# KorAP/Datok

Measured on AMD Instinct MI355X. Metric: input MB/s tokenized, tokenizer_de.matok, higher is better.
Workload: dtype u32 table cells, u8 symbol codes; 1 GPU; tokenizer_de.matok, 4096 equal-length 4096 B synthetic German docs per batch (BASELINE.json configs[1]); table_layout=matrix: state-major fused u32 cells, docs_per_gpu=4096, doc_bytes=4096, parallelism=documents sharded over 1 GPU(s), no data-path collective, batches_in_flight=3, inputs=one per batch in flight (generator seeds 2, 3, 4 on rank 0)

## Files before the change

### datok_amd/csrc/dtk_symbolize.hip

```cpp
#include "dtk_device.h"

__device__ __forceinline__ uint32_t go_width(uint32_t b0, uint32_t b1, uint32_t b2, uint32_t b3, uint32_t avail) {
  const uint32_t c1 = (b1 & 0xC0u) == 0x80u, c2 = (b2 & 0xC0u) == 0x80u, c3 = (b3 & 0xC0u) == 0x80u;
  const uint32_t two = (uint32_t)(b0 - 0xC2u < 0x1Eu) & (uint32_t)(avail >= 2u) & c1;
  const uint32_t lo3 = b0 == 0xE0u ? 0xA0u : 0x80u, hi3 = b0 == 0xEDu ? 0x9Fu : 0xBFu;
  const uint32_t three = (uint32_t)((b0 & 0xF0u) == 0xE0u) & (uint32_t)(avail >= 3u) & (uint32_t)(b1 >= lo3) &
                         (uint32_t)(b1 <= hi3) & c2;
  const uint32_t lo4 = b0 == 0xF0u ? 0x90u : 0x80u, hi4 = b0 == 0xF4u ? 0x8Fu : 0xBFu;
  const uint32_t four = (uint32_t)(b0 - 0xF0u <= 4u) & (uint32_t)(avail >= 4u) & (uint32_t)(b1 >= lo4) &
                        (uint32_t)(b1 <= hi4) & c2 & c3;
  return 1u + two + 2u * three + 3u * four;
}


#define SYM_BLOCK_BYTES DTK_SYM_BLOCK_BYTES
#define SYM_SIG_LDS 64u
#define SYM_HALF 1024u
#define SYM_THREADS (WAVE * (SYM_BLOCK_BYTES / SYM_HALF))
#define SYM_DOFF (SYM_BLOCK_BYTES / 16u)
#define SYM_FAR 0x10000u

__device__ __forceinline__ void sym_clear_acc(uint4 *__restrict__ acc, uint32_t acc16) {
  if (!acc) return;
  const uint4 z = make_uint4(0u, 0u, 0u, 0u);
  constexpr uint32_t kept16 = offsetof(DtkTotalsDev, invalid_epoch) / 16u;
  constexpr uint32_t flags8 = offsetof(DtkTotalsDev, any_irregular) / 8u;
  for (uint32_t i = blockIdx.x * SYM_THREADS + threadIdx.x; i < acc16; i += gridDim.x * SYM_THREADS) {
    if (i == kept16) reinterpret_cast<unsigned long long *>(acc)[flags8] = 0ull;
    else acc[i] = z;
  }
}

__device__ __forceinline__ void sym_clear_events(uint32_t *__restrict__ ev_bits, uint32_t bit_words, uint64_t block_start,
                                                 uint32_t n_here, uint32_t d_lo, uint32_t d_hi) {
  if (!ev_bits) return;
  const uint64_t ga = block_start + d_lo, gb = block_start + n_here + d_hi + 1u;
  const uint32_t wa = blockIdx.x == 0 ? 0u : (uint32_t)(ga >> 5);
  uint32_t wb = (uint32_t)((gb + 31u) >> 5);
  if (wb > bit_words || blockIdx.x == gridDim.x - 1) wb = bit_words;
  for (uint32_t w = wa + threadIdx.x; w < wb; w += SYM_THREADS)
#pragma unroll
    for (uint32_t k = 0; k < EVB_KINDS; k++) ev_bits[(size_t)k * bit_words + w] = 0u;
}

__device__ __forceinline__ void sym_saw_invalid(bool bad, unsigned long long *__restrict__ n_invalid, unsigned long long epoch) {
  if (__ballot(bad) != 0ull && lane_id() == 0 &&
      __hip_atomic_load(n_invalid, __ATOMIC_RELAXED, __HIP_MEMORY_SCOPE_AGENT) != epoch)
    atomicMax(n_invalid, epoch);
}


__device__ __forceinline__ uint32_t sym_gather7(uint32_t x) {
  uint32_t t = x & 0x80808080u;
  t |= t << 7;
  t |= t << 14;
  return t >> 28;
}
__device__ __forceinline__ uint32_t sym_bytes_of7(uint32_t m) { return (m << 1) - (m >> 7); }
__device__ __forceinline__ uint32_t sym_spread7(uint32_t nib) {
  uint32_t t = nib | (nib << 7);
  t |= t << 14;
  return (t & 0x01010101u) << 7;
}
__device__ __forceinline__ uint32_t sym_window(uint32_t w0, uint32_t w1, uint32_t w2, uint32_t w3, uint32_t nx,
                                                        uint32_t p) {
  const bool k1 = (p & 4u) != 0u, k2 = (p & 8u) != 0u;
  const uint32_t lo = k2 ? (k1 ? w3 : w2) : (k1 ? w1 : w0), hi = k2 ? (k1 ? nx : w3) : (k1 ? w2 : w1);
  return __builtin_amdgcn_alignbyte(hi, lo, p & 3u);
}
__device__ __forceinline__ void sym_patch(uint32_t &w0, uint32_t &w1, uint32_t &w2, uint32_t &w3, uint32_t p,
                                                   uint32_t code) {
  const uint32_t sh = 8u * (p & 3u), keep = ~(0xFFu << sh), c = code << sh, k = p >> 2;
  w0 = k == 0u ? (w0 & keep) | c : w0;
  w1 = k == 1u ? (w1 & keep) | c : w1;
  w2 = k == 2u ? (w2 & keep) | c : w2;
  w3 = k == 3u ? (w3 & keep) | c : w3;
}
__device__ __forceinline__ uint32_t sym_rune(uint32_t x, uint32_t w) {
  const uint32_t b0 = x & 0xFFu, b1 = (x >> 8) & 0x3Fu, b2 = (x >> 16) & 0x3Fu, b3 = (x >> 24) & 0x3Fu;
  const uint32_t r2 = ((b0 & 0x1Fu) << 6) | b1;
  const uint32_t r3 = ((b0 & 0x0Fu) << 12) | (b1 << 6) | b2;
  const uint32_t r4 = ((b0 & 0x07u) << 18) | (b1 << 12) | (b2 << 6) | b3;
  return w == 2u ? r2 : (w == 3u ? r3 : r4);
}

template <bool ALIGNED4>
__global__ __launch_bounds__(SYM_THREADS) void k_symbolize8(const uint8_t *__restrict__ text,
                                                     const uint64_t *__restrict__ doc_off,
                                                     uint32_t n_docs, uint64_t total, DtkSigmaDev sig,
                                                     uint8_t *__restrict__ sym8,
                                                     const uint32_t *__restrict__ blk_doc,
                                                     unsigned long long *__restrict__ n_invalid,
                                                     uint32_t *__restrict__ rs_bits,
                                                     uint32_t *__restrict__ ev_bits, uint32_t bit_words,
                                                     uint4 *__restrict__ acc, uint32_t acc16,
                                                     unsigned long long epoch) {
  sym_clear_acc(acc, acc16);
  __shared__ uint32_t s_lat[64];
  __shared__ uint32_t s_runes[SYM_SIG_LDS];
  __shared__ uint8_t s_codes[SYM_SIG_LDS];
  __shared__ uint64_t s_doff[SYM_DOFF];
  const uint32_t tid = threadIdx.x, lane = tid & (WAVE - 1u);
  const uint64_t block_start = (uint64_t)blockIdx.x * SYM_BLOCK_BYTES;
  const uint32_t n_here = (uint32_t)min((uint64_t)SYM_BLOCK_BYTES, total - block_start);
  const uint32_t i0 = tid * 16u;
  const uint64_t g0 = block_start + i0;

  auto load4 = [&](uint64_t g) -> uint32_t {
    uint32_t x = 0;
    if (ALIGNED4) {
      if (g < total) {
        x = *reinterpret_cast<const uint32_t *>(text + g);
        if (total - g < 4u) x &= (1u << (8u * (uint32_t)(total - g))) - 1u;
      }
    } else {
      for (int k = 0; k < 4; k++)
        if (g + k < total) x |= (uint32_t)text[g + k] << (8 * k);
    }
    return x;
  };
  uint32_t w0, w1, w2, w3, halo = 0;
  if (ALIGNED4 && total - block_start >= SYM_BLOCK_BYTES + 4u) {
    const uint32_t *t4 = reinterpret_cast<const uint32_t *>(text + g0);
    w0 = t4[0]; w1 = t4[1]; w2 = t4[2]; w3 = t4[3];
    if (lane == 0 && g0 >= 4u) halo = t4[-1];
    if (lane == WAVE - 1u) halo = t4[4];
  } else {
    w0 = load4(g0); w1 = load4(g0 + 4u); w2 = load4(g0 + 8u); w3 = load4(g0 + 12u);
    if (lane == 0 && g0 >= 4u) halo = load4(g0 - 4u);
    if (lane == WAVE - 1u) halo = load4(g0 + 16u);
  }

  const bool sig_lds = sig.n_runes < SYM_SIG_LDS;
  if (tid < 64u) s_lat[tid] = reinterpret_cast<const uint32_t *>(sig.code_lt256)[tid];
  if (sig_lds && tid < SYM_SIG_LDS) {
    s_runes[tid] = tid < sig.n_runes ? sig.runes[tid] : 0xFFFFFFFFu;
    if (tid < sig.n_runes) s_codes[tid] = sig.code_runes[tid];
  }
  const uint32_t d_lo = blk_doc[blockIdx.x];
  const uint32_t d_hi = min(blk_doc[blockIdx.x + 1], n_docs - 1);
  const uint32_t n_off = d_hi - d_lo + 2u;
  if (n_off <= SYM_DOFF && tid < n_off) s_doff[tid] = doc_off[d_lo + tid];
  const uint64_t lo_start = doc_off[d_lo], lo_end = doc_off[d_lo + 1];
  const uint32_t lo_end_rel = (uint32_t)min(lo_end - block_start, (uint64_t)SYM_FAR);
  sym_clear_events(ev_bits, bit_words, block_start, n_here, d_lo, d_hi);
  __syncthreads();

  if ((tid & ~(WAVE - 1u)) * 16u >= n_here) return;
  auto doc_end_rel = [&](uint32_t pos) -> uint32_t {
    const uint64_t g = block_start + pos;
    uint64_t dend;
    if (n_off <= SYM_DOFF) {
      uint32_t lo = 0, hi = n_off - 1u;
      while (hi - lo > 1u) {
        const uint32_t mid = lo + ((hi - lo) >> 1);
        if (s_doff[mid] <= g) lo = mid; else hi = mid;
      }
      dend = s_doff[lo + 1u];
    } else {
      dend = doc_off[doc_of(doc_off, d_lo, d_hi + 1, g) + 1u];
    }
    return (uint32_t)min(dend - block_start, (uint64_t)SYM_FAR);
  };

  const uint32_t nval = i0 < n_here ? min(n_here - i0, 16u) : 0u;
  uint32_t covered = 0;
  if (__ballot(((w0 | w1 | w2 | w3) & 0x80808080u) != 0u) != 0ull) {
    const uint32_t nx = (uint32_t)__builtin_amdgcn_update_dpp((int)halo, (int)w0, 0x130, 0xF, 0xF, false);
    const uint32_t hi16 = sym_gather7(w0) | (sym_gather7(w1) << 4) | (sym_gather7(w2) << 8) | (sym_gather7(w3) << 12);
    uint32_t lead = sym_gather7(w0 & (w0 << 1)) | (sym_gather7(w1 & (w1 << 1)) << 4) |
                    (sym_gather7(w2 & (w2 << 1)) << 8) | (sym_gather7(w3 & (w3 << 1)) << 12);
    const uint32_t cont16 = hi16 & ~lead;
    const uint32_t c0 = w0 & ~(w0 << 1) & 0x80808080u, c1 = w1 & ~(w1 << 1) & 0x80808080u,
                   c2 = w2 & ~(w2 << 1) & 0x80808080u, c3 = w3 & ~(w3 << 1) & 0x80808080u;
    const uint32_t invalid_code = sig.code_fffd1;
    bool bad = false;
    uint32_t dend = lo_end_rel;
    auto width_at = [&](uint32_t x, uint32_t pos) -> uint32_t {
      if (pos >= dend) dend = doc_end_rel(pos);
      return go_width(x & 0xFFu, (x >> 8) & 0xFFu, (x >> 16) & 0xFFu, x >> 24, min(dend - pos, 4u));
    };
    uint32_t spill0 = 0;
    if (lane == 0 && (cont16 & 1u) && g0 >= 4u) {
      const uint32_t k = halo >= 0xC0000000u ? 1u : ((halo & 0x00C00000u) == 0x00C00000u ? 2u : ((halo & 0x0000C000u) == 0x0000C000u ? 3u : 0u));
      if (k) {
        const uint32_t x = __builtin_amdgcn_alignbyte(w0, halo, 4u - k);
        const uint64_t g = g0 - k;
        uint64_t de = lo_end;
        if (g < lo_start) de = doc_off[doc_of(doc_off, 0, d_lo, g) + 1u];
        else if (g >= lo_end) de = block_start + doc_end_rel(i0 - k);
        const uint32_t w = go_width(x & 0xFFu, (x >> 8) & 0xFFu, (x >> 16) & 0xFFu, x >> 24, (uint32_t)min(de - g, (uint64_t)4u));
        spill0 = w > k ? (1u << (w - k)) - 1u : 0u;
      }
    }
    for (; __builtin_amdgcn_ballot_w64(lead != 0u) != 0ull; lead &= lead - 1u) {
      if (lead == 0u) continue;
      const uint32_t p = (uint32_t)__builtin_ctz(lead);
      const uint32_t x = sym_window(w0, w1, w2, w3, nx, p);
      const uint32_t w = width_at(x, i0 + p);
      uint32_t code = invalid_code;
      if (w >= 2u) {
        const uint32_t rune = sym_rune(x, w);
        if (rune < 256u) {
          code = (s_lat[rune >> 2] >> (8u * (rune & 3u))) & 0xFFu;
        } else {
          code = w == 2u ? sig.code_ident[2] : (w == 3u ? sig.code_ident[3] : sig.code_ident[4]);
          if (sig_lds) {
            uint32_t n = 0;
#pragma unroll
            for (uint32_t step = SYM_SIG_LDS / 2u; step; step >>= 1) n += s_runes[n + step - 1u] <= rune ? step : 0u;
            if (n && s_runes[n - 1u] == rune) code = s_codes[n - 1u];
          } else {
            uint32_t base = 0;
            for (uint32_t len = sig.n_runes; len > 1u;) {
              const uint32_t half = len >> 1;
              base = sig.runes[base + half] <= rune ? base + half : base;
              len -= half;
            }
            if (sig.runes[base] == rune) code = sig.code_runes[base];
          }
        }
      }
      sym_patch(w0, w1, w2, w3, p, code);
      covered |= ((1u << w) - 2u) << p;
      bad |= w == 1u;
    }
    uint32_t spill = (uint32_t)__builtin_amdgcn_update_dpp(0, (int)(covered >> 16), 0x138, 0xF, 0xF, false);
    if (lane == 0) spill = spill0;
    covered = (covered | spill) & 0xFFFFu;
    static_assert(DTK_SYM_CONT == 0xFFu, "a continuation byte becomes DTK_SYM_CONT by setting all its bits");
    w0 |= sym_bytes_of7(c0); w1 |= sym_bytes_of7(c1); w2 |= sym_bytes_of7(c2); w3 |= sym_bytes_of7(c3);
    const uint32_t stray = cont16 & ~covered;
    if (__ballot(stray != 0u) != 0ull) {
      const uint32_t flip = (DTK_SYM_CONT ^ invalid_code) * 0x01010101u;
      w0 ^= sym_bytes_of7(sym_spread7(stray & 15u)) & flip;
      w1 ^= sym_bytes_of7(sym_spread7((stray >> 4) & 15u)) & flip;
      w2 ^= sym_bytes_of7(sym_spread7((stray >> 8) & 15u)) & flip;
      w3 ^= sym_bytes_of7(sym_spread7(stray >> 12)) & flip;
      bad |= stray != 0u;
    }
    sym_saw_invalid(bad, n_invalid, epoch);
  }

  if (nval == 16u && ((reinterpret_cast<uintptr_t>(sym8) + block_start) & 15u) == 0) {
    *reinterpret_cast<uint4 *>(sym8 + g0) = make_uint4(w0, w1, w2, w3);
  } else {
#pragma unroll
    for (uint32_t j = 0; j < 16u; j++) {
      const uint32_t wj = j < 4u ? w0 : (j < 8u ? w1 : (j < 12u ? w2 : w3));
      if (j < nval) sym8[g0 + j] = (uint8_t)(wj >> (8u * (j & 3u)));
    }
  }
  const uint32_t starts = ((1u << nval) - 1u) & ~covered;
  const uint32_t upper = (uint32_t)__builtin_amdgcn_update_dpp(0, (int)starts, 0x101, 0xF, 0xF, true);
  if (!(lane & 1u) && nval) rs_bits[(block_start >> 5) + (tid >> 1)] = starts | (upper << 16);
}

#define SYM_TILE 512u

template <bool ALIGNED4>
__global__ __launch_bounds__(SYM_THREADS) void k_symbolize16(const uint8_t *__restrict__ text,
                                                    const uint64_t *__restrict__ doc_off,
                                                    uint32_t n_docs, uint64_t total, DtkSigmaDev sig,
                                                    uint16_t *__restrict__ sym,
                                                    const uint32_t *__restrict__ blk_doc,
                                                    unsigned long long *__restrict__ n_invalid,
                                                    uint32_t *__restrict__ rs_bits,
                                                    uint32_t *__restrict__ ev_bits, uint32_t bit_words,
                                                    uint4 *__restrict__ acc, uint32_t acc16,
                                                    unsigned long long epoch) {
  sym_clear_acc(acc, acc16);
  __shared__ uint32_t s_rs[SYM_BLOCK_BYTES / 32];
  __shared__ uint16_t lut[128];
  __shared__ uint16_t lat[256];
  __shared__ uint32_t s_runes[SYM_SIG_LDS];
  __shared__ uint16_t s_syms[SYM_SIG_LDS];
  __shared__ uint32_t s_txt[SYM_BLOCK_BYTES / 4 + 4];
  __shared__ uint16_t s_qs[SYM_BLOCK_BYTES / SYM_HALF][SYM_HALF];
  __shared__ uint64_t s_doff[SYM_DOFF];
  const uint32_t tid = threadIdx.x, lane = tid & (WAVE - 1u), half = tid >> 6;
  uint16_t *s_q = s_qs[half];
  const bool sig_lds = sig.n_runes <= SYM_SIG_LDS;
  for (uint32_t i = tid; i < SYM_BLOCK_BYTES / 32; i += SYM_THREADS) s_rs[i] = 0;
  for (uint32_t i = tid; i < 256u; i += SYM_THREADS) {
    const uint32_t e = (sig.ascii[i] & DTK_SYM_MASK) | (i == DTK_EOT ? (1u << DTK_SYM_CLS_SHIFT) : 0u);
    lat[i] = (uint16_t)e;
    if (i < 128u) lut[i] = (uint16_t)(e | (1u << DTK_SYM_W_SHIFT));
    if (sig_lds && i < sig.n_runes) { s_runes[i] = sig.runes[i]; s_syms[i] = sig.syms[i]; }
  }
  const uint64_t block_start = (uint64_t)blockIdx.x * SYM_BLOCK_BYTES;
  const uint32_t n_here = (uint32_t)min((uint64_t)SYM_BLOCK_BYTES, total - block_start);
  const uint32_t d_lo = blk_doc[blockIdx.x];
  const uint32_t d_hi = min(blk_doc[blockIdx.x + 1], n_docs - 1);
  const uint32_t n_off = d_hi - d_lo + 2u;
  if (n_off <= SYM_DOFF && tid < n_off) s_doff[tid] = doc_off[d_lo + tid];
  {
    auto load4 = [&](uint64_t g) -> uint32_t {
      if (ALIGNED4) return g < total ? *reinterpret_cast<const uint32_t *>(text + g) : 0u;
      uint32_t x = 0;
      for (int k = 0; k < 4; k++)
        if (g + k < total) x |= (uint32_t)text[g + k] << (8 * k);
      return x;
    };
    uint32_t v[SYM_BLOCK_BYTES / 4 / SYM_THREADS];
#pragma unroll
    for (uint32_t r = 0; r < SYM_BLOCK_BYTES / 4 / SYM_THREADS; r++) v[r] = load4(block_start + (r * SYM_THREADS + tid) * 4u);
    uint32_t halo = 0;
    if (tid == 0 && block_start >= 4) halo = load4(block_start - 4);
    if (tid == 1) halo = load4(block_start + SYM_BLOCK_BYTES);
#pragma unroll
    for (uint32_t r = 0; r < SYM_BLOCK_BYTES / 4 / SYM_THREADS; r++) s_txt[1 + r * SYM_THREADS + tid] = v[r];
    if (tid == 0) s_txt[0] = halo;
    if (tid == 1) s_txt[1 + SYM_BLOCK_BYTES / 4] = halo;
  }
  __syncthreads();
  const uint8_t *__restrict__ sb = reinterpret_cast<const uint8_t *>(s_txt) + 4;

  const uint64_t lo_start = doc_off[d_lo], lo_end = doc_off[d_lo + 1];
  sym_clear_events(ev_bits, bit_words, block_start, n_here, d_lo, d_hi);
  const bool sym16 = ((reinterpret_cast<uintptr_t>(sym) + 2ull * block_start) & 15u) == 0;

  if (half * SYM_HALF < n_here) {
    uint32_t qn = 0;
    auto light = [&](auto full_tag, uint32_t it) {
      constexpr bool FULL = decltype(full_tag)::value;
      const uint32_t i0 = half * SYM_HALF + it * SYM_TILE + lane * 8u;
      const uint32_t w0 = s_txt[1 + (i0 >> 2)], w1 = s_txt[2 + (i0 >> 2)];
      uint32_t left = 8u;
      if (!FULL) left = i0 < n_here ? (n_here - i0 >= 8u ? 8u : n_here - i0) : 0u;
      const uint32_t e0 = lut[w0 & 0x7Fu], e1 = lut[(w0 >> 8) & 0x7Fu];
      const uint32_t e2 = lut[(w0 >> 16) & 0x7Fu], e3 = lut[(w0 >> 24) & 0x7Fu];
      const uint32_t e4 = lut[w1 & 0x7Fu], e5 = lut[(w1 >> 8) & 0x7Fu];
      const uint32_t e6 = lut[(w1 >> 16) & 0x7Fu], e7 = lut[(w1 >> 24) & 0x7Fu];
      if (FULL || (left == 8u && sym16)) {
        *reinterpret_cast<uint4 *>(sym + block_start + i0) =
            make_uint4(e0 | (e1 << 16), e2 | (e3 << 16), e4 | (e5 << 16), e6 | (e7 << 16));
      } else {
        const uint32_t o[8] = {e0, e1, e2, e3, e4, e5, e6, e7};
        for (uint32_t j = 0; j < left; j++) sym[block_start + i0 + j] = (uint16_t)o[j];
      }
      auto nib = [](uint32_t x) { return ((x >> 7) & 1u) | ((x >> 14) & 2u) | ((x >> 21) & 4u) | ((x >> 28) & 8u); };
      const uint32_t valid = FULL ? 0xFFu : ((1u << left) - 1u);
      const uint32_t rare = (nib(w0 & 0x80808080u) | (nib(w1 & 0x80808080u) << 4)) & valid;
      const uint32_t asc = ~rare & valid;
      if (asc) atomicOr(&s_rs[i0 >> 5], asc << (i0 & 31u));
      const uint32_t cnt = (uint32_t)__popc(rare);
      const unsigned long long b0 = __ballot(cnt & 1u), b1 = __ballot(cnt & 2u), b2 = __ballot(cnt & 4u),
                               b3 = __ballot(cnt & 8u);
      if ((b0 | b1 | b2 | b3) == 0ull) return;
      const unsigned long long lt = lanemask_lt();
      uint32_t slot = qn + popc(b0 & lt) + 2u * popc(b1 & lt) + 4u * popc(b2 & lt) + 8u * popc(b3 & lt);
      qn += popc(b0) + 2u * popc(b1) + 4u * popc(b2) + 8u * popc(b3);
      for (uint32_t m = rare; __builtin_amdgcn_ballot_w64(m != 0u) != 0ull; m &= m - 1u)
        if (m) s_q[slot++] = (uint16_t)(i0 + (uint32_t)__builtin_ctz(m));
    };
    const bool full_block = n_here == SYM_BLOCK_BYTES && sym16;
#pragma unroll 1
    for (uint32_t it = 0; it < SYM_HALF / SYM_TILE; it++) {
      if (half * SYM_HALF + it * SYM_TILE >= n_here) break;
      if (full_block) light(std::true_type{}, it); else light(std::false_type{}, it);
    }
    __builtin_amdgcn_fence(__ATOMIC_ACQ_REL, "wavefront");
    __builtin_amdgcn_wave_barrier();
    const uint32_t nq = qn;
    if (nq) __builtin_amdgcn_s_waitcnt(0);

    for (uint32_t q0 = 0; q0 < nq; q0 += WAVE) {
      bool bad = false;
      if (q0 + lane < nq) {
        const uint32_t pos = s_q[q0 + lane];
        const uint64_t g = block_start + pos;
        uint64_t dstart = lo_start, dend = lo_end;
        if (g >= lo_end) {
          if (n_off <= SYM_DOFF) {
            uint32_t lo = 0, hi = n_off - 1u;
            while (hi - lo > 1u) {
              const uint32_t mid = lo + ((hi - lo) >> 1);
              if (s_doff[mid] <= g) lo = mid; else hi = mid;
            }
            dstart = s_doff[lo]; dend = s_doff[lo + 1u];
          } else {
            const uint32_t d = doc_of(doc_off, d_lo, d_hi + 1, g);
            dstart = doc_off[d]; dend = doc_off[d + 1];
          }
        }
        const uint64_t l64 = dend - g, b64 = g - dstart;
        const uint32_t avail = l64 > 8 ? 8u : (uint32_t)l64, back = b64 > 3 ? 3u : (uint32_t)b64;
        uint32_t bb[7];
#pragma unroll
        for (int k = 0; k < 7; k++) {
          const int o = k - 3;
          const bool in = o < 0 ? (uint32_t)(-o) <= back : (uint32_t)o < avail;
          bb[k] = in ? (uint32_t)sb[(int)pos + o] : 0u;
        }
        const uint32_t b0 = bb[3], b1 = bb[4], b2 = bb[5], b3 = bb[6];
        const uint32_t n1 = (uint32_t)((bb[2] & 0xC0u) != 0x80u), n2 = (uint32_t)((bb[1] & 0xC0u) != 0x80u),
                       n3 = (uint32_t)((bb[0] & 0xC0u) != 0x80u);
        const uint32_t in1 = (uint32_t)(back >= 1u), in2 = (uint32_t)(back >= 2u), in3 = (uint32_t)(back >= 3u);
        const uint32_t cont = (uint32_t)((b0 & 0xC0u) == 0x80u);
        const uint32_t k1 = cont & in1 & n1, k2 = cont & in2 & (n1 ^ 1u) & n2, k3 = cont & in3 & (n1 ^ 1u) & (n2 ^ 1u) & n3;
        const uint32_t k = k1 + 2u * k2 + 3u * k3;
        const uint32_t c0 = k3 ? bb[0] : (k2 ? bb[1] : (k1 ? bb[2] : b0)), c1 = k3 ? bb[1] : (k2 ? bb[2] : (k1 ? b0 : b1));
        const uint32_t c2 = k3 ? bb[2] : (k2 ? b0 : (k1 ? b1 : b2)), c3 = k3 ? b0 : (k2 ? b1 : (k1 ? b2 : b3));
        const uint32_t wseq = go_width(c0, c1, c2, c3, avail + k);
        const uint32_t start = k ? (uint32_t)(wseq <= k) : 1u;
        const uint32_t wd = cont ? 1u : wseq;
        const uint32_t r2 = ((b0 & 0x1Fu) << 6) | (b1 & 0x3Fu);
        const uint32_t r3 = ((b0 & 0x0Fu) << 12) | ((b1 & 0x3Fu) << 6) | (b2 & 0x3Fu);
        const uint32_t r4 = ((b0 & 0x07u) << 18) | ((b1 & 0x3Fu) << 12) | ((b2 & 0x3Fu) << 6) | (b3 & 0x3Fu);
        const uint32_t rune = wd == 1 ? 0xFFFDu : (wd == 2 ? r2 : (wd == 3 ? r3 : r4));
        uint32_t a_cls;
        if (rune < 256u) {
          a_cls = lat[rune];
        } else {
          int l = 0, h = (int)sig.n_runes - 1;
          a_cls = (sig.identity & DTK_SYM_MASK) | (3u << DTK_SYM_CLS_SHIFT);
          while (l <= h) {
            const int m = (l + h) >> 1;
            const uint32_t r = sig_lds ? s_runes[m] : sig.runes[m];
            if (r == rune) {
              a_cls = ((sig_lds ? (uint32_t)s_syms[m] : (uint32_t)sig.syms[m]) & DTK_SYM_MASK) | (2u << DTK_SYM_CLS_SHIFT);
              break;
            }
            if (r < rune) l = m + 1; else h = m - 1;
          }
        }
        sym[g] = (uint16_t)(a_cls | (start ? wd << DTK_SYM_W_SHIFT : 0u));
        if (start) atomicOr(&s_rs[pos >> 5], 1u << (pos & 31u));
        bad = start && wd == 1u;
      }
      sym_saw_invalid(bad, n_invalid, epoch);
    }
  }
  __syncthreads();
  for (uint32_t i = tid; i < SYM_BLOCK_BYTES / 32; i += SYM_THREADS)
    if (i * 32u < n_here) rs_bits[(block_start >> 5) + i] = s_rs[i];
}


extern "C" int dtk_launch_symbolize(const uint8_t *text, const uint64_t *doc_off, uint32_t n_docs,
                                    uint64_t total, const DtkSigmaDev *sig, void *sym, int padded,
                                    const uint32_t *blk_doc, unsigned long long *n_invalid, uint32_t *rs_bits,
                                    uint32_t *ev_bits, uint32_t bit_words, void *acc, uint64_t acc_bytes,
                                    uint64_t epoch, void *stream) {
  if (total == 0 || n_docs == 0) return 0;
  const uint32_t blocks = (uint32_t)((total + SYM_BLOCK_BYTES - 1) / SYM_BLOCK_BYTES);
  const bool al4 = (((uintptr_t)text) & 3u) == 0 && (padded || (total & 3u) == 0);
  auto go = [&](auto k, auto *out) {
    hipLaunchKernelGGL(k, dim3(blocks), dim3(SYM_THREADS), 0, (hipStream_t)stream, text, doc_off, n_docs,
                       total, *sig, out, blk_doc, n_invalid, rs_bits, ev_bits, bit_words, (uint4 *)acc, (uint32_t)(acc_bytes / 16),
                       (unsigned long long)epoch);
  };
  if (sig->n_codes) { if (al4) go(k_symbolize8<true>, (uint8_t *)sym); else go(k_symbolize8<false>, (uint8_t *)sym); }
  else { if (al4) go(k_symbolize16<true>, (uint16_t *)sym); else go(k_symbolize16<false>, (uint16_t *)sym); }
  return (int)hipGetLastError();
}
```

Baseline: 191,400 MB/s.

## Widen symbolize8 to 32 bytes per lane with a wave-uniform two-byte fast path

The 8-bit symbolize kernel now has each lane process 32 input bytes instead of 16, which halves the thread count per block and lets each lane write its rs_bits word directly instead of combining two lanes through DPP. The lead-byte loop adds a path for iterations where every pending lane has a valid two-byte UTF-8 sequence, skipping the full width and rune decode. The patch and continuation-byte masking helpers are simplified into XOR and multiply-free forms. The cost is higher register pressure and longer per-lane serial loops over lead bytes, which may reduce occupancy and latency hiding.

```diff
diff --git a/datok_amd/csrc/dtk_symbolize.hip b/datok_amd/csrc/dtk_symbolize.hip
--- a/datok_amd/csrc/dtk_symbolize.hip
+++ b/datok_amd/csrc/dtk_symbolize.hip
@@ -17,20 +17,25 @@
 #define SYM_SIG_LDS 64u
 #define SYM_HALF 1024u
 #define SYM_THREADS (WAVE * (SYM_BLOCK_BYTES / SYM_HALF))
+#define SYM8_LANE 32u
+#define SYM8_WAVE (WAVE * SYM8_LANE)
+#define SYM8_THREADS (WAVE * (SYM_BLOCK_BYTES / SYM8_WAVE))
 #define SYM_DOFF (SYM_BLOCK_BYTES / 16u)
 #define SYM_FAR 0x10000u
 
+template <uint32_t THREADS = SYM_THREADS>
 __device__ __forceinline__ void sym_clear_acc(uint4 *__restrict__ acc, uint32_t acc16) {
   if (!acc) return;
   const uint4 z = make_uint4(0u, 0u, 0u, 0u);
   constexpr uint32_t kept16 = offsetof(DtkTotalsDev, invalid_epoch) / 16u;
   constexpr uint32_t flags8 = offsetof(DtkTotalsDev, any_irregular) / 8u;
-  for (uint32_t i = blockIdx.x * SYM_THREADS + threadIdx.x; i < acc16; i += gridDim.x * SYM_THREADS) {
+  for (uint32_t i = blockIdx.x * THREADS + threadIdx.x; i < acc16; i += gridDim.x * THREADS) {
     if (i == kept16) reinterpret_cast<unsigned long long *>(acc)[flags8] = 0ull;
     else acc[i] = z;
   }
 }
 
+template <uint32_t THREADS = SYM_THREADS>
 __device__ __forceinline__ void sym_clear_events(uint32_t *__restrict__ ev_bits, uint32_t bit_words, uint64_t block_start,
                                                  uint32_t n_here, uint32_t d_lo, uint32_t d_hi) {
   if (!ev_bits) return;
@@ -38,7 +43,7 @@
   const uint32_t wa = blockIdx.x == 0 ? 0u : (uint32_t)(ga >> 5);
   uint32_t wb = (uint32_t)((gb + 31u) >> 5);
   if (wb > bit_words || blockIdx.x == gridDim.x - 1) wb = bit_words;
-  for (uint32_t w = wa + threadIdx.x; w < wb; w += SYM_THREADS)
+  for (uint32_t w = wa + threadIdx.x; w < wb; w += THREADS)
 #pragma unroll
     for (uint32_t k = 0; k < EVB_KINDS; k++) ev_bits[(size_t)k * bit_words + w] = 0u;
 }
@@ -56,25 +61,24 @@
   t |= t << 14;
   return t >> 28;
 }
-__device__ __forceinline__ uint32_t sym_bytes_of7(uint32_t m) { return (m << 1) - (m >> 7); }
-__device__ __forceinline__ uint32_t sym_spread7(uint32_t nib) {
+__device__ __forceinline__ uint32_t sym_bytes_of4(uint32_t nib) {
   uint32_t t = nib | (nib << 7);
   t |= t << 14;
-  return (t & 0x01010101u) << 7;
-}
-__device__ __forceinline__ uint32_t sym_window(uint32_t w0, uint32_t w1, uint32_t w2, uint32_t w3, uint32_t nx,
-                                                        uint32_t p) {
-  const bool k1 = (p & 4u) != 0u, k2 = (p & 8u) != 0u;
-  const uint32_t lo = k2 ? (k1 ? w3 : w2) : (k1 ? w1 : w0), hi = k2 ? (k1 ? nx : w3) : (k1 ? w2 : w1);
+  t &= 0x01010101u;
+  return (t << 8) - t;
+}
+__device__ __forceinline__ uint32_t sym_window(const uint32_t (&w)[8], uint32_t nx, uint32_t p) {
+  const bool k4 = (p & 16u) != 0u, k2 = (p & 8u) != 0u, k1 = (p & 4u) != 0u;
+  const uint32_t a0 = k4 ? w[4] : w[0], a1 = k4 ? w[5] : w[1], a2 = k4 ? w[6] : w[2], a3 = k4 ? w[7] : w[3],
+                 a4 = k4 ? nx : w[4];
+  const uint32_t b0 = k2 ? a2 : a0, b1 = k2 ? a3 : a1, b2 = k2 ? a4 : a2;
+  const uint32_t lo = k1 ? b1 : b0, hi = k1 ? b2 : b1;
   return __builtin_amdgcn_alignbyte(hi, lo, p & 3u);
 }
-__device__ __forceinline__ void sym_patch(uint32_t &w0, uint32_t &w1, uint32_t &w2, uint32_t &w3, uint32_t p,
-                                                   uint32_t code) {
-  const uint32_t sh = 8u * (p & 3u), keep = ~(0xFFu << sh), c = code << sh, k = p >> 2;
-  w0 = k == 0u ? (w0 & keep) | c : w0;
-  w1 = k == 1u ? (w1 & keep) | c : w1;
-  w2 = k == 2u ? (w2 & keep) | c : w2;
-  w3 = k == 3u ? (w3 & keep) | c : w3;
+__device__ __forceinline__ void sym_patch(uint32_t (&w)[8], uint32_t p, uint32_t was, uint32_t code) {
+  const uint32_t flip = (was ^ code) << (8u * (p & 3u)), k = p >> 2;
+#pragma unroll
+  for (uint32_t j = 0; j < 8u; j++) w[j] ^= k == j ? flip : 0u;
 }
 __device__ __forceinline__ uint32_t sym_rune(uint32_t x, uint32_t w) {
   const uint32_t b0 = x & 0xFFu, b1 = (x >> 8) & 0x3Fu, b2 = (x >> 16) & 0x3Fu, b3 = (x >> 24) & 0x3Fu;
@@ -85,7 +89,7 @@
 }
 
 template <bool ALIGNED4>
-__global__ __launch_bounds__(SYM_THREADS) void k_symbolize8(const uint8_t *__restrict__ text,
+__global__ __launch_bounds__(SYM8_THREADS) void k_symbolize8(const uint8_t *__restrict__ text,
                                                      const uint64_t *__restrict__ doc_off,
                                                      uint32_t n_docs, uint64_t total, DtkSigmaDev sig,
                                                      uint8_t *__restrict__ sym8,
@@ -95,7 +99,7 @@
                                                      uint32_t *__restrict__ ev_bits, uint32_t bit_words,
                                                      uint4 *__restrict__ acc, uint32_t acc16,
                                                      unsigned long long epoch) {
-  sym_clear_acc(acc, acc16);
+  sym_clear_acc<SYM8_THREADS>(acc, acc16);
   __shared__ uint32_t s_lat[64];
   __shared__ uint32_t s_runes[SYM_SIG_LDS];
   __shared__ uint8_t s_codes[SYM_SIG_LDS];
@@ -103,7 +107,7 @@
   const uint32_t tid = threadIdx.x, lane = tid & (WAVE - 1u);
   const uint64_t block_start = (uint64_t)blockIdx.x * SYM_BLOCK_BYTES;
   const uint32_t n_here = (uint32_t)min((uint64_t)SYM_BLOCK_BYTES, total - block_start);
-  const uint32_t i0 = tid * 16u;
+  const uint32_t i0 = tid * SYM8_LANE;
   const uint64_t g0 = block_start + i0;
 
   auto load4 = [&](uint64_t g) -> uint32_t {
@@ -119,16 +123,18 @@
     }
     return x;
   };
-  uint32_t w0, w1, w2, w3, halo = 0;
+  uint32_t w[8], halo = 0;
   if (ALIGNED4 && total - block_start >= SYM_BLOCK_BYTES + 4u) {
     const uint32_t *t4 = reinterpret_cast<const uint32_t *>(text + g0);
-    w0 = t4[0]; w1 = t4[1]; w2 = t4[2]; w3 = t4[3];
+#pragma unroll
+    for (uint32_t j = 0; j < 8u; j++) w[j] = t4[j];
     if (lane == 0 && g0 >= 4u) halo = t4[-1];
-    if (lane == WAVE - 1u) halo = t4[4];
+    if (lane == WAVE - 1u) halo = t4[8];
   } else {
-    w0 = load4(g0); w1 = load4(g0 + 4u); w2 = load4(g0 + 8u); w3 = load4(g0 + 12u);
+#pragma unroll
+    for (uint32_t j = 0; j < 8u; j++) w[j] = load4(g0 + 4u * j);
     if (lane == 0 && g0 >= 4u) halo = load4(g0 - 4u);
-    if (lane == WAVE - 1u) halo = load4(g0 + 16u);
+    if (lane == WAVE - 1u) halo = load4(g0 + SYM8_LANE);
   }
 
   const bool sig_lds = sig.n_runes < SYM_SIG_LDS;
@@ -140,13 +146,17 @@
   const uint32_t d_lo = blk_doc[blockIdx.x];
   const uint32_t d_hi = min(blk_doc[blockIdx.x + 1], n_docs - 1);
   const uint32_t n_off = d_hi - d_lo + 2u;
-  if (n_off <= SYM_DOFF && tid < n_off) s_doff[tid] = doc_off[d_lo + tid];
+  static_assert(SYM_DOFF == 2u * SYM8_THREADS, "two offsets per thread fill s_doff");
+  if (n_off <= SYM_DOFF) {
+    if (tid < n_off) s_doff[tid] = doc_off[d_lo + tid];
+    if (tid + SYM8_THREADS < n_off) s_doff[tid + SYM8_THREADS] = doc_off[d_lo + tid + SYM8_THREADS];
+  }
   const uint64_t lo_start = doc_off[d_lo], lo_end = doc_off[d_lo + 1];
   const uint32_t lo_end_rel = (uint32_t)min(lo_end - block_start, (uint64_t)SYM_FAR);
-  sym_clear_events(ev_bits, bit_words, block_start, n_here, d_lo, d_hi);
+  sym_clear_events<SYM8_THREADS>(ev_bits, bit_words, block_start, n_here, d_lo, d_hi);
   __syncthreads();
 
-  if ((tid & ~(WAVE - 1u)) * 16u >= n_here) return;
+  if ((tid & ~(WAVE - 1u)) * SYM8_LANE >= n_here) return;
   auto doc_end_rel = [&](uint32_t pos) -> uint32_t {
     const uint64_t g = block_start + pos;
     uint64_t dend;
@@ -163,97 +173,118 @@
     return (uint32_t)min(dend - block_start, (uint64_t)SYM_FAR);
   };
 
-  const uint32_t nval = i0 < n_here ? min(n_here - i0, 16u) : 0u;
-  uint32_t covered = 0;
-  if (__ballot(((w0 | w1 | w2 | w3) & 0x80808080u) != 0u) != 0ull) {
-    const uint32_t nx = (uint32_t)__builtin_amdgcn_update_dpp((int)halo, (int)w0, 0x130, 0xF, 0xF, false);
-    const uint32_t hi16 = sym_gather7(w0) | (sym_gather7(w1) << 4) | (sym_gather7(w2) << 8) | (sym_gather7(w3) << 12);
-    uint32_t lead = sym_gather7(w0 & (w0 << 1)) | (sym_gather7(w1 & (w1 << 1)) << 4) |
-                    (sym_gather7(w2 & (w2 << 1)) << 8) | (sym_gather7(w3 & (w3 << 1)) << 12);
-    const uint32_t cont16 = hi16 & ~lead;
-    const uint32_t c0 = w0 & ~(w0 << 1) & 0x80808080u, c1 = w1 & ~(w1 << 1) & 0x80808080u,
-                   c2 = w2 & ~(w2 << 1) & 0x80808080u, c3 = w3 & ~(w3 << 1) & 0x80808080u;
+  const uint32_t nval = i0 < n_here ? min(n_here - i0, SYM8_LANE) : 0u;
+  unsigned long long covered = 0;
+  uint32_t any = 0;
+#pragma unroll
+  for (uint32_t j = 0; j < 8u; j++) any |= w[j];
+  if (__ballot((any & 0x80808080u) != 0u) != 0ull) {
+    const uint32_t nx = (uint32_t)__builtin_amdgcn_update_dpp((int)halo, (int)w[0], 0x130, 0xF, 0xF, false);
+    uint32_t hi32 = 0, lead = 0;
+#pragma unroll
+    for (uint32_t j = 0; j < 8u; j++) {
+      hi32 |= sym_gather7(w[j]) << (4u * j);
+      lead |= sym_gather7(w[j] & (w[j] << 1)) << (4u * j);
+    }
+    const uint32_t cont32 = hi32 & ~lead;
     const uint32_t invalid_code = sig.code_fffd1;
     bool bad = false;
     uint32_t dend = lo_end_rel;
-    auto width_at = [&](uint32_t x, uint32_t pos) -> uint32_t {
-      if (pos >= dend) dend = doc_end_rel(pos);
-      return go_width(x & 0xFFu, (x >> 8) & 0xFFu, (x >> 16) & 0xFFu, x >> 24, min(dend - pos, 4u));
+    auto code_ge256 = [&](uint32_t rune, uint32_t ident) -> uint32_t {
+      uint32_t code = ident;
+      if (sig_lds) {
+        uint32_t n = 0;
+#pragma unroll
+        for (uint32_t step = SYM_SIG_LDS / 2u; step; step >>= 1) n += s_runes[n + step - 1u] <= rune ? step : 0u;
+        if (n && s_runes[n - 1u] == rune) code = s_codes[n - 1u];
+      } else {
+        uint32_t base = 0;
+        for (uint32_t len = sig.n_runes; len > 1u;) {
+          const uint32_t half = len >> 1;
+          base = sig.runes[base + half] <= rune ? base + half : base;
+          len -= half;
+        }
+        if (sig.runes[base] == rune) code = sig.code_runes[base];
+      }
+      return code;
     };
     uint32_t spill0 = 0;
-    if (lane == 0 && (cont16 & 1u) && g0 >= 4u) {
+    if (lane == 0 && (cont32 & 1u) && g0 >= 4u) {
       const uint32_t k = halo >= 0xC0000000u ? 1u : ((halo & 0x00C00000u) == 0x00C00000u ? 2u : ((halo & 0x0000C000u) == 0x0000C000u ? 3u : 0u));
       if (k) {
-        const uint32_t x = __builtin_amdgcn_alignbyte(w0, halo, 4u - k);
+        const uint32_t x = __builtin_amdgcn_alignbyte(w[0], halo, 4u - k);
         const uint64_t g = g0 - k;
         uint64_t de = lo_end;
         if (g < lo_start) de = doc_off[doc_of(doc_off, 0, d_lo, g) + 1u];
         else if (g >= lo_end) de = block_start + doc_end_rel(i0 - k);
-        const uint32_t w = go_width(x & 0xFFu, (x >> 8) & 0xFFu, (x >> 16) & 0xFFu, x >> 24, (uint32_t)min(de - g, (uint64_t)4u));
-        spill0 = w > k ? (1u << (w - k)) - 1u : 0u;
-      }
-    }
-    for (; __builtin_amdgcn_ballot_w64(lead != 0u) != 0ull; lead &= lead - 1u) {
+        const uint32_t wd = go_width(x & 0xFFu, (x >> 8) & 0xFFu, (x >> 16) & 0xFFu, x >> 24, (uint32_t)min(de - g, (uint64_t)4u));
+        spill0 = wd > k ? (1u << (wd - k)) - 1u : 0u;
+      }
+    }
+    for (;; lead &= lead - 1u) {
+      uint32_t p = 0, x = 0, avail = 0;
+      bool two = false;
+      if (lead != 0u) {
+        p = (uint32_t)__builtin_ctz(lead);
+        x = sym_window(w, nx, p);
+        if (i0 + p >= dend) dend = doc_end_rel(i0 + p);
+        avail = min(dend - (i0 + p), 4u);
+        two = ((x & 0xFFu) - 0xC2u < 0x1Eu) & ((x & 0xC000u) == 0x8000u) & (avail >= 2u);
+      }
+      const unsigned long long pending = __builtin_amdgcn_ballot_w64(lead != 0u);
+      if (pending == 0ull) break;
+      if (__builtin_amdgcn_ballot_w64(two) == pending) {
+        if (lead != 0u) {
+          const uint32_t rune = ((x & 0x1Fu) << 6) | ((x >> 8) & 0x3Fu);
+          const uint32_t code = rune < 256u ? (s_lat[rune >> 2] >> (8u * (rune & 3u))) & 0xFFu
+                                            : code_ge256(rune, sig.code_ident[2]);
+          sym_patch(w, p, x & 0xFFu, code);
+          covered |= 2ull << p;
+        }
+        continue;
+      }
       if (lead == 0u) continue;
-      const uint32_t p = (uint32_t)__builtin_ctz(lead);
-      const uint32_t x = sym_window(w0, w1, w2, w3, nx, p);
-      const uint32_t w = width_at(x, i0 + p);
+      const uint32_t wd = go_width(x & 0xFFu, (x >> 8) & 0xFFu, (x >> 16) & 0xFFu, x >> 24, avail);
       uint32_t code = invalid_code;
-      if (w >= 2u) {
-        const uint32_t rune = sym_rune(x, w);
-        if (rune < 256u) {
-          code = (s_lat[rune >> 2] >> (8u * (rune & 3u))) & 0xFFu;
-        } else {
-          code = w == 2u ? sig.code_ident[2] : (w == 3u ? sig.code_ident[3] : sig.code_ident[4]);
-          if (sig_lds) {
-            uint32_t n = 0;
-#pragma unroll
-            for (uint32_t step = SYM_SIG_LDS / 2u; step; step >>= 1) n += s_runes[n + step - 1u] <= rune ? step : 0u;
-            if (n && s_runes[n - 1u] == rune) code = s_codes[n - 1u];
-          } else {
-            uint32_t base = 0;
-            for (uint32_t len = sig.n_runes; len > 1u;) {
-              const uint32_t half = len >> 1;
-              base = sig.runes[base + half] <= rune ? base + half : base;
-              len -= half;
-            }
-            if (sig.runes[base] == rune) code = sig.code_runes[base];
-          }
-        }
-      }
-      sym_patch(w0, w1, w2, w3, p, code);
-      covered |= ((1u << w) - 2u) << p;
-      bad |= w == 1u;
-    }
-    uint32_t spill = (uint32_t)__builtin_amdgcn_update_dpp(0, (int)(covered >> 16), 0x138, 0xF, 0xF, false);
+      if (wd >= 2u) {
+        const uint32_t rune = sym_rune(x, wd);
+        code = rune < 256u ? (s_lat[rune >> 2] >> (8u * (rune & 3u))) & 0xFFu
+                           : code_ge256(rune, wd == 2u ? sig.code_ident[2] : (wd == 3u ? sig.code_ident[3] : sig.code_ident[4]));
+      }
+      sym_patch(w, p, x & 0xFFu, code);
+      covered |= (unsigned long long)((1u << wd) - 2u) << p;
+      bad |= wd == 1u;
+    }
+    uint32_t spill = (uint32_t)__builtin_amdgcn_update_dpp(0, (int)(uint32_t)(covered >> 32), 0x138, 0xF, 0xF, false);
     if (lane == 0) spill = spill0;
-    covered = (covered | spill) & 0xFFFFu;
+    covered = (uint32_t)covered | spill;
     static_assert(DTK_SYM_CONT == 0xFFu, "a continuation byte becomes DTK_SYM_CONT by setting all its bits");
-    w0 |= sym_bytes_of7(c0); w1 |= sym_bytes_of7(c1); w2 |= sym_bytes_of7(c2); w3 |= sym_bytes_of7(c3);
-    const uint32_t stray = cont16 & ~covered;
+#pragma unroll
+    for (uint32_t j = 0; j < 8u; j++) w[j] |= sym_bytes_of4((cont32 >> (4u * j)) & 15u);
+    const uint32_t stray = cont32 & ~(uint32_t)covered;
     if (__ballot(stray != 0u) != 0ull) {
       const uint32_t flip = (DTK_SYM_CONT ^ invalid_code) * 0x01010101u;
-      w0 ^= sym_bytes_of7(sym_spread7(stray & 15u)) & flip;
-      w1 ^= sym_bytes_of7(sym_spread7((stray >> 4) & 15u)) & flip;
-      w2 ^= sym_bytes_of7(sym_spread7((stray >> 8) & 15u)) & flip;
-      w3 ^= sym_bytes_of7(sym_spread7(stray >> 12)) & flip;
+#pragma unroll
+      for (uint32_t j = 0; j < 8u; j++) w[j] ^= sym_bytes_of4((stray >> (4u * j)) & 15u) & flip;
       bad |= stray != 0u;
     }
     sym_saw_invalid(bad, n_invalid, epoch);
   }
 
-  if (nval == 16u && ((reinterpret_cast<uintptr_t>(sym8) + block_start) & 15u) == 0) {
-    *reinterpret_cast<uint4 *>(sym8 + g0) = make_uint4(w0, w1, w2, w3);
-  } else {
-#pragma unroll
-    for (uint32_t j = 0; j < 16u; j++) {
-      const uint32_t wj = j < 4u ? w0 : (j < 8u ? w1 : (j < 12u ? w2 : w3));
-      if (j < nval) sym8[g0 + j] = (uint8_t)(wj >> (8u * (j & 3u)));
-    }
-  }
-  const uint32_t starts = ((1u << nval) - 1u) & ~covered;
-  const uint32_t upper = (uint32_t)__builtin_amdgcn_update_dpp(0, (int)starts, 0x101, 0xF, 0xF, true);
-  if (!(lane & 1u) && nval) rs_bits[(block_start >> 5) + (tid >> 1)] = starts | (upper << 16);
+  const bool al16 = ((reinterpret_cast<uintptr_t>(sym8) + block_start) & 15u) == 0;
+#pragma unroll
+  for (uint32_t h = 0; h < 2u; h++) {
+    const uint32_t nv = nval > 16u * h ? min(nval - 16u * h, 16u) : 0u;
+    if (nv == 16u && al16) {
+      *reinterpret_cast<uint4 *>(sym8 + g0 + 16u * h) = make_uint4(w[4u * h], w[4u * h + 1u], w[4u * h + 2u], w[4u * h + 3u]);
+    } else {
+#pragma unroll
+      for (uint32_t j = 0; j < 16u; j++)
+        if (j < nv) sym8[g0 + 16u * h + j] = (uint8_t)(w[4u * h + (j >> 2)] >> (8u * (j & 3u)));
+    }
+  }
+  const uint32_t valid = nval >= 32u ? 0xFFFFFFFFu : (1u << nval) - 1u;
+  if (nval) rs_bits[(block_start >> 5) + tid] = valid & ~(uint32_t)covered;
 }
 
 #define SYM_TILE 512u
@@ -446,12 +477,12 @@
   if (total == 0 || n_docs == 0) return 0;
   const uint32_t blocks = (uint32_t)((total + SYM_BLOCK_BYTES - 1) / SYM_BLOCK_BYTES);
   const bool al4 = (((uintptr_t)text) & 3u) == 0 && (padded || (total & 3u) == 0);
-  auto go = [&](auto k, auto *out) {
-    hipLaunchKernelGGL(k, dim3(blocks), dim3(SYM_THREADS), 0, (hipStream_t)stream, text, doc_off, n_docs,
+  auto go = [&](auto k, auto *out, uint32_t threads) {
+    hipLaunchKernelGGL(k, dim3(blocks), dim3(threads), 0, (hipStream_t)stream, text, doc_off, n_docs,
                        total, *sig, out, blk_doc, n_invalid, rs_bits, ev_bits, bit_words, (uint4 *)acc, (uint32_t)(acc_bytes / 16),
                        (unsigned long long)epoch);
   };
-  if (sig->n_codes) { if (al4) go(k_symbolize8<true>, (uint8_t *)sym); else go(k_symbolize8<false>, (uint8_t *)sym); }
-  else { if (al4) go(k_symbolize16<true>, (uint16_t *)sym); else go(k_symbolize16<false>, (uint16_t *)sym); }
+  if (sig->n_codes) { if (al4) go(k_symbolize8<true>, (uint8_t *)sym, SYM8_THREADS); else go(k_symbolize8<false>, (uint8_t *)sym, SYM8_THREADS); }
+  else { if (al4) go(k_symbolize16<true>, (uint16_t *)sym, SYM_THREADS); else go(k_symbolize16<false>, (uint16_t *)sym, SYM_THREADS); }
   return (int)hipGetLastError();
 }
```

New measurement: 192,700 MB/s (median of 5 runs). Within noise of the previous version (+0.7%).
